# ZhenghaoFei/visual_odom

Hardware: NVIDIA H100
Metric: stereo frames/sec at 1241x376, 2000 feats; LK kernel HBM GB/s vs roofline (higher is better)
Workload: dtype u8/i32 fixed point + f32 (LK), f64 (pose)

## Files before the change

visual_odom_b200/csrc/ctx.cu:

```cuda
#include "ctx.h"
#include <string.h>
#include <stdlib.h>

void vo_set_error(vo_ctx* ctx, const char* fmt, ...)
{
    if (!ctx) return;
    va_list ap;
    va_start(ap, fmt);
    vsnprintf(ctx->err, sizeof(ctx->err), fmt, ap);
    va_end(ap);
}

extern "C" void vo_default_params(vo_params* p)
{
    p->fast_threshold = 20;
    p->fast_nonmax = 1;
    p->lk_win = 21;
    p->lk_max_level = 3;
    p->lk_max_iters = 30;
    p->lk_epsilon = 0.01;
    p->lk_min_eig = 0.001;
    p->circ_threshold = 0;
    p->pnp_iterations = 500;
    p->pnp_reproj_error = 0.5f;
// ... 260 lines not shown
    for (auto& p : ctx->pending)
        if (p.active) {
            VO_CUDA_CHECK(cudaEventSynchronize(p.done));
            p.active = false;
        }
    if (ctx->seq_inflight > 0 && ctx->side_stream[0]) VO_CUDA_CHECK(cudaStreamSynchronize(ctx->side_stream[0]));
    return VO_OK;
}

void vo_drop_graphs(vo_ctx* ctx)
{
    for (auto& g : ctx->graphs) cudaGraphExecDestroy(g.exec);
    ctx->graphs.clear();
}

void vo_set_calibration(vo_ctx* ctx, const float P_l[12], const float P_r[12])
{
    const bool same = ctx->have_P && memcmp(ctx->P_l, P_l, 12 * sizeof(float)) == 0 && memcmp(ctx->P_r, P_r, 12 * sizeof(float)) == 0;
    if (same) return;
    vo_drop_graphs(ctx);
    memcpy(ctx->P_l, P_l, 12 * sizeof(float));
    memcpy(ctx->P_r, P_r, 12 * sizeof(float));
    ctx->have_P = true;
}

void vo_free_state(vo_ctx* ctx)
{
    vo_drop_graphs(ctx);
    for (void* p : ctx->allocs) cudaFree(p);
    ctx->allocs.clear();
    if (ctx->d_seq_state) cudaFree(ctx->d_seq_state);
    ctx->d_seq_state = nullptr; ctx->seq_n_cap = 0;
    ctx->d_feat_pts = nullptr; ctx->d_feat_ages = nullptr; ctx->d_feat_cnt = ctx->d_bucket = ctx->d_seq_err = ctx->d_seq_live = nullptr;
    ctx->d_out = nullptr; ctx->out_stride = 0; ctx->out_per = 0;
    ctx->w = ctx->h = ctx->units = 0;
}

template <typename T>
static cudaError_t dalloc(vo_ctx* ctx, T** p, size_t count)
{
    void* q = nullptr;
    cudaError_t e = cudaMalloc(&q, count * sizeof(T) + 256);
    if (e == cudaSuccess) { ctx->allocs.push_back(q); *p = (T*)q; }
    return e;
}

typedef CUresult (*PFN_encodeTiled)(CUtensorMap*, CUtensorMapDataType, cuuint32_t, void*, const cuuint64_t*,
                                    const cuuint64_t*, const cuuint32_t*, const cuuint32_t*, CUtensorMapInterleave,
                                    CUtensorMapSwizzle, CUtensorMapL2promotion, CUtensorMapFloatOOBfill);

static int encode_maps(vo_ctx* ctx)
{
    void* fn = nullptr;
    cudaDriverEntryPointQueryResult qres;
    VO_CUDA_CHECK(cudaGetDriverEntryPoint("cuTensorMapEncodeTiled", &fn, cudaEnableDefault, &qres));
    if (!fn || qres != cudaDriverEntryPointSuccess) {
        vo_set_error(ctx, "cuTensorMapEncodeTiled not available from the driver");
        return VO_E_CUDA;
    }
    PFN_encodeTiled enc = (PFN_encodeTiled)fn;
    const int n_img = ctx->units * 4;
    for (int l = 0; l < ctx->pg.nlevels; l++) {
        const LevelGeom& g = ctx->pg.lv[l];
        {
            cuuint64_t dims[3] = {(cuuint64_t)g.pitch, (cuuint64_t)g.hp, (cuuint64_t)n_img};
            cuuint64_t strides[2] = {(cuuint64_t)g.pitch, (cuuint64_t)g.plane};
            cuuint32_t box_i[3] = {48, 22, 1}, box_j[3] = {48, 32, 1};
            cuuint32_t estr[3] = {1, 1, 1};
            CUresult r = enc(&ctx->maps.img_i[l], CU_TENSOR_MAP_DATA_TYPE_UINT8, 3, g.img, dims, strides, box_i, estr,
                             CU_TENSOR_MAP_INTERLEAVE_NONE, CU_TENSOR_MAP_SWIZZLE_NONE,
                             CU_TENSOR_MAP_L2_PROMOTION_NONE, CU_TENSOR_MAP_FLOAT_OOB_FILL_NONE);
            if (r == CUDA_SUCCESS)
                r = enc(&ctx->maps.img_j[l], CU_TENSOR_MAP_DATA_TYPE_UINT8, 3, g.img, dims, strides, box_j, estr,
                        CU_TENSOR_MAP_INTERLEAVE_NONE, CU_TENSOR_MAP_SWIZZLE_NONE,
                        CU_TENSOR_MAP_L2_PROMOTION_NONE, CU_TENSOR_MAP_FLOAT_OOB_FILL_NONE);
            if (r != CUDA_SUCCESS) { vo_set_error(ctx, "cuTensorMapEncodeTiled(u8 level %d) failed: %d", l, (int)r); return VO_E_CUDA; }
        }
        {
            cuuint64_t dims[3] = {(cuuint64_t)g.pitch, (cuuint64_t)g.hp, (cuuint64_t)n_img};
            cuuint64_t strides[2] = {(cuuint64_t)g.pitch * 4, (cuuint64_t)g.plane * 4};
            cuuint32_t box[3] = {28, 22, 1};
            cuuint32_t estr[3] = {1, 1, 1};
            CUresult r = enc(&ctx->maps.der[l], CU_TENSOR_MAP_DATA_TYPE_UINT32, 3, g.der, dims, strides, box, estr,
                             CU_TENSOR_MAP_INTERLEAVE_NONE, CU_TENSOR_MAP_SWIZZLE_NONE,
                             CU_TENSOR_MAP_L2_PROMOTION_NONE, CU_TENSOR_MAP_FLOAT_OOB_FILL_NONE);
            if (r != CUDA_SUCCESS) { vo_set_error(ctx, "cuTensorMapEncodeTiled(deriv level %d) failed: %d", l, (int)r); return VO_E_CUDA; }
        }
    }
    return VO_OK;
}

int vo_ensure_state(vo_ctx* ctx, int w, int h, int units, int )
{
    if (w <= 0 || h <= 0 || units <= 0) { vo_set_error(ctx, "bad geometry %dx%d units=%d", w, h, units); return VO_E_INVALID; }
    if (ctx->w == w && ctx->h == h && ctx->units >= units) return VO_OK;
    VO_CUDA_CHECK(cudaSetDevice(ctx->device));
    { int drc = vo_drain_pending(ctx); if (drc) return drc; }
    VO_CUDA_CHECK(cudaStreamSynchronize(ctx->stream));
    vo_free_state(ctx);
    const int n_img = units * 4;
    const int cap = ctx->cap;
    PyrGeom& pg = ctx->pg;
    memset(&pg, 0, sizeof(pg));
    int cw = w, ch = h;
    for (int l = 0; l <= ctx->p.lk_max_level; l++) {
        if (l > 0) {
            int nw = (cw + 1) / 2, nh = (ch + 1) / 2;
            if (nw <= VO_WIN || nh <= VO_WIN) break;
            cw = nw; ch = nh;
        }
        LevelGeom& g = pg.lv[l];
        g.w = cw; g.h = ch;
        g.pitch = ((cw + 2 * VO_PAD) + 63) / 64 * 64;
        g.hp = ch + 2 * VO_PAD;
        g.plane = (size_t)g.pitch * g.hp;
        VO_CUDA_CHECK(dalloc(ctx, &g.img, g.plane * n_img));
        VO_CUDA_CHECK(dalloc(ctx, &g.der, g.plane * n_img));
        VO_CUDA_CHECK(cudaMemsetAsync(g.img, 0, g.plane * n_img, ctx->stream));
        VO_CUDA_CHECK(cudaMemsetAsync(g.der, 0, g.plane * n_img * sizeof(uint32_t), ctx->stream));
        pg.nlevels = l + 1;
    }
    pg.n_img = n_img;
    VO_CUDA_CHECK(dalloc(ctx, &ctx->d_raw, (size_t)n_img * w * h));
    VO_CUDA_CHECK(dalloc(ctx, &ctx->d_raw_tab, (size_t)n_img));
    VO_CUDA_CHECK(dalloc(ctx, &ctx->d_ingest_tab, (size_t)n_img));
    {
        std::vector<const uint8_t*> tab(n_img);
        for (int i = 0; i < n_img; i++) tab[i] = ctx->d_raw + (size_t)i * w * h;
        VO_CUDA_CHECK(cudaMemcpyAsync(ctx->d_raw_tab, tab.data(), n_img * sizeof(uint8_t*), cudaMemcpyHostToDevice, ctx->stream));
        VO_CUDA_CHECK(cudaStreamSynchronize(ctx->stream));
    }
    const size_t uc = (size_t)units * cap;
    VO_CUDA_CHECK(dalloc(ctx, &ctx->d_pts_in, uc));
    VO_CUDA_CHECK(dalloc(ctx, &ctx->d_npts, (size_t)units));
    VO_CUDA_CHECK(dalloc(ctx, &ctx->d_pts_out, 4 * uc));
    VO_CUDA_CHECK(dalloc(ctx, &ctx->d_status, 4 * uc));
    VO_CUDA_CHECK(dalloc(ctx, &ctx->d_err, 4 * uc));
    VO_CUDA_CHECK(dalloc(ctx, &ctx->d_lk_progress, uc));
    VO_CUDA_CHECK(cudaMemsetAsync(ctx->d_lk_progress, 0, uc * sizeof(int), ctx->stream));
    VO_CUDA_CHECK(dalloc(ctx, &ctx->d_ages_in, uc));
    VO_CUDA_CHECK(dalloc(ctx, &ctx->d_ages_out, uc));
    VO_CUDA_CHECK(dalloc(ctx, &ctx->d_kept5, 5 * uc));
    VO_CUDA_CHECK(dalloc(ctx, &ctx->d_idx3, uc));
    VO_CUDA_CHECK(dalloc(ctx, &ctx->d_n3, (size_t)units));
    VO_CUDA_CHECK(dalloc(ctx, &ctx->d_valid4, 4 * uc));
    VO_CUDA_CHECK(dalloc(ctx, &ctx->d_idx5, uc));
    VO_CUDA_CHECK(dalloc(ctx, &ctx->d_n5, (size_t)units));
    {
        const long iw = w > 6 ? w - 6 : 0, ih = h > 6 ? h - 6 : 0;
        const long bound = ctx->p.fast_nonmax ? ((iw + 1) / 2) * ((ih + 1) / 2) : iw * ih;
        if (bound > (1L << 30)) { vo_set_error(ctx, "%dx%d: too many possible FAST corners", w, h); return VO_E_CAPACITY; }
        ctx->corner_cap = bound > 0 ? (int)bound : 1;
    }
    VO_CUDA_CHECK(dalloc(ctx, &ctx->d_score, (size_t)units * w * h));
    VO_CUDA_CHECK(dalloc(ctx, &ctx->d_rowbuf, (size_t)units * h * w));
    VO_CUDA_CHECK(dalloc(ctx, &ctx->d_rowcount, (size_t)units * h));
    VO_CUDA_CHECK(dalloc(ctx, &ctx->d_rowoff, (size_t)units * h));
    VO_CUDA_CHECK(dalloc(ctx, &ctx->d_ndet, (size_t)units));
    VO_CUDA_CHECK(dalloc(ctx, &ctx->d_corners, (size_t)units * ctx->corner_cap));
    VO_CUDA_CHECK(dalloc(ctx, &ctx->d_resp, (size_t)units * ctx->corner_cap));
    VO_CUDA_CHECK(dalloc(ctx, &ctx->d_want, (size_t)units));
    const size_t its = (size_t)ctx->p.pnp_iterations;
    VO_CUDA_CHECK(dalloc(ctx, &ctx->d_X, uc));
    VO_CUDA_CHECK(dalloc(ctx, &ctx->d_tprev, (size_t)units * 3));
    VO_CUDA_CHECK(dalloc(ctx, &ctx->d_pnp_state, (size_t)units));
    VO_CUDA_CHECK(dalloc(ctx, &ctx->d_subsets, (size_t)units * its * 5));
    VO_CUDA_CHECK(dalloc(ctx, &ctx->d_models, (size_t)units * its * 12));
    VO_CUDA_CHECK(dalloc(ctx, &ctx->d_counts, (size_t)units * its));
    VO_CUDA_CHECK(dalloc(ctx, &ctx->d_inliers, uc));
    VO_CUDA_CHECK(dalloc(ctx, &ctx->d_results, (size_t)units));
    ctx->feat_cap = ctx->corner_cap + cap;
    ctx->seq_active = false;
    VO_CUDA_CHECK(cudaMemsetAsync(ctx->d_results, 0, (size_t)units * sizeof(vo_unit_result_dev), ctx->stream));
    VO_CUDA_CHECK(cudaMemsetAsync(ctx->d_tprev, 0, (size_t)units * 3 * sizeof(double), ctx->stream));
    ctx->w = w; ctx->h = h; ctx->units = units;
    int rc = encode_maps(ctx);
    if (rc != VO_OK) { vo_free_state(ctx); return rc; }
    VO_CUDA_CHECK(cudaStreamSynchronize(ctx->stream));
    return VO_OK;
}

int vo_run_pyramid(vo_ctx* ctx, int plane0, int nplanes, cudaStream_t s)
{
    PyrGeom pg = ctx->pg;
    pg.n_img = nplanes;
    for (int l = 0; l < pg.nlevels; l++) {
        pg.lv[l].img += (size_t)plane0 * pg.lv[l].plane;
        pg.lv[l].der += (size_t)plane0 * pg.lv[l].plane;
    }
    ctx->launches += vo_launch_pyramid(pg, ctx->d_raw_tab + plane0, ctx->w, s);
    VO_CUDA_CHECK(cudaGetLastError());
    return VO_OK;
}

int vo_run_lk(vo_ctx* ctx, const View& v, int ncalls, const int* img_prev, const int* img_next, bool want_err)
{
    int rc = vo_run_pyramid(ctx, v.u0 * ctx->imgs_per_unit, v.n * ctx->imgs_per_unit, v.s);
    if (rc) return rc;
    return vo_run_lk_ring(ctx, v, ncalls, img_prev, img_next, want_err);
}

int vo_run_lk_ring(vo_ctx* ctx, const View& v, int ncalls, const int* img_prev, const int* img_next, bool want_err)
{
    const int ipu = ctx->imgs_per_unit;
    const size_t uo = (size_t)v.u0 * ctx->cap;
    const PyrGeom& pg = ctx->pg;

    LkArgs a;
    memset(&a, 0, sizeof(a));
    a.n_units = v.n;
    a.cap = ctx->cap;
    a.n_pts = ctx->d_npts + v.u0;
    a.imgs_per_unit = ipu;
    a.img_plane0 = v.plane0 >= 0 ? v.plane0 : v.u0 * ipu;
    a.ncalls = ncalls;
    for (int c = 0; c < ncalls; c++) { a.img_prev[c] = img_prev[c]; a.img_next[c] = img_next[c]; }
    a.nlevels = pg.nlevels;
    for (int l = 0; l < pg.nlevels; l++) { a.lw[l] = pg.lv[l].w; a.lh[l] = pg.lv[l].h; }
    a.max_iters = ctx->p.lk_max_iters;
    double eps = ctx->p.lk_epsilon;
    if (eps < 0.) eps = 0.; if (eps > 10.) eps = 10.;
    a.eps2 = eps * eps;
    a.min_eig = ctx->p.lk_min_eig;
    a.pts_in = ctx->d_pts_in + uo;
    a.pts_out = ctx->d_pts_out + uo;
    a.status_out = ctx->d_status + uo;
    a.err_out = want_err ? ctx->d_err + uo : nullptr;
    a.call_stride = (size_t)ctx->units * ctx->cap;
    a.use_tma = ctx->lk_use_tma ? 1 : 0;
    for (int l = 0; l < pg.nlevels; l++) {
        a.img_base[l] = ctx->pg.lv[l].img; a.der_base[l] = ctx->pg.lv[l].der;
        a.pitch[l] = pg.lv[l].pitch; a.plane[l] = pg.lv[l].plane;
    }

    cudaEvent_t e0 = nullptr, e1 = nullptr;
    if (ctx->lk_timing) {
        if (ctx->ev_used + 2 > ctx->ev_pool.size()) {
            cudaEvent_t a0, a1;
            VO_CUDA_CHECK(cudaEventCreate(&a0));
            VO_CUDA_CHECK(cudaEventCreate(&a1));
            ctx->ev_pool.push_back(a0); ctx->ev_pool.push_back(a1);
        }
        e0 = ctx->ev_pool[ctx->ev_used]; e1 = ctx->ev_pool[ctx->ev_used + 1];
        ctx->ev_used += 2;
        VO_CUDA_CHECK(cudaEventRecord(e0, v.s));
    }
    {
        size_t qi = 0;
        while (qi < ctx->lk_queue_streams.size() && ctx->lk_queue_streams[qi] != v.s) qi++;
        if (qi == ctx->lk_queue_streams.size()) {
            if (qi >= LK_QUEUES) { vo_set_error(ctx, "more than %d streams launch the LK kernel", LK_QUEUES); return VO_E_CAPACITY; }
            ctx->lk_queue_streams.push_back(v.s);
        }
        a.queue = ctx->d_lk_queue + 2 * qi;
        a.per_unit = ctx->lk_per_unit > 0 && ctx->lk_per_unit < ctx->cap ? ctx->lk_per_unit : ctx->cap;
        a.progress = ctx->d_lk_progress + uo;
        {
            int lk_sms = ctx->sm_count;
            for (int c = 0; c < VO_LANES; c++) if (ctx->part_on && v.s == ctx->part_lk_stream[c]) lk_sms = ctx->part_lk_sms;
            const long resident_warps = (long)lk_sms * vo_lk_ctas_per_sm(ctx->lk_ctas_per_sm) * LK_WARPS_PER_CTA;
            const bool big = (long)a.n_units * a.per_unit > resident_warps;
            a.span = ctx->lk_span > 0 ? ctx->lk_span : (big ? 2 : 0);
            a.quota = big ? ctx->lk_quota : 0;
        }
        int lk_sms = ctx->sm_count;
        for (int c = 0; c < VO_LANES; c++) if (ctx->part_on && v.s == ctx->part_lk_stream[c]) lk_sms = ctx->part_lk_sms;
        VO_CUDA_CHECK(vo_launch_lk_ring(ctx->maps, a, lk_sms, ctx->lk_ctas_per_sm, v.s));
    }
    ctx->launches += 1;
    if (e1) VO_CUDA_CHECK(cudaEventRecord(e1, v.s));
    return VO_OK;
}

int vo_run_filter(vo_ctx* ctx, const View& v, bool with_ages)
{
    const size_t uo = (size_t)v.u0 * ctx->cap;
    FilterArgs f;
    memset(&f, 0, sizeof(f));
    f.cap = ctx->cap;
    f.call_stride = (size_t)ctx->units * ctx->cap;
    f.circ_threshold = ctx->p.circ_threshold;
    f.n_pts = ctx->d_npts + v.u0;
    f.pts_in = ctx->d_pts_in + uo;
    f.pts_out = ctx->d_pts_out + uo;
    f.status = ctx->d_status + uo;
    f.ages_in = with_ages ? ctx->d_ages_in + uo : nullptr;
    f.ages_out = ctx->d_ages_out + uo;
    f.kept5 = ctx->d_kept5 + uo;
    f.idx3 = ctx->d_idx3 + uo;
    f.n3 = ctx->d_n3 + v.u0;
    f.valid4 = ctx->d_valid4 + uo;
    f.idx5 = ctx->d_idx5 + uo;
    f.n5 = ctx->d_n5 + v.u0;
    VO_CUDA_CHECK(vo_launch_ring_filter(f, v.n, v.s));
    ctx->launches += 1;
    return VO_OK;
}

int vo_run_fast(vo_ctx* ctx, const View& v, int plane_in_unit, bool want_resp)
{
    FastArgs a;
    memset(&a, 0, sizeof(a));
    const size_t plane = (size_t)ctx->w * ctx->h;
    a.n_units = v.n;
    a.img_tab = ctx->d_raw_tab + (size_t)(v.plane0 >= 0 ? v.plane0 : v.u0 * ctx->imgs_per_unit) + plane_in_unit;
    a.img_stride_idx = ctx->imgs_per_unit;
    a.w = ctx->w; a.h = ctx->h; a.pitch = ctx->w;
    a.threshold = ctx->p.fast_threshold; a.nonmax = ctx->p.fast_nonmax;
    a.score = ctx->d_score + v.u0 * plane; a.score_plane = plane;
    a.rowbuf = ctx->d_rowbuf + v.u0 * plane; a.rowcap = ctx->w;
    a.rowcount = ctx->d_rowcount + (size_t)v.u0 * ctx->h; a.rowoff = ctx->d_rowoff + (size_t)v.u0 * ctx->h;
    a.n_det = ctx->d_ndet + v.u0;
    a.corners = ctx->d_corners + (size_t)v.u0 * ctx->corner_cap;
    a.resp = want_resp ? ctx->d_resp + (size_t)v.u0 * ctx->corner_cap : nullptr;
    a.corner_cap = ctx->corner_cap;
    ctx->launches += vo_launch_fast(a, v.s);
    VO_CUDA_CHECK(cudaGetLastError());
    return VO_OK;
}

int vo_run_select(vo_ctx* ctx, const View& v)
{
    ctx->launches += vo_launch_select(ctx->d_corners + (size_t)v.u0 * ctx->corner_cap, ctx->corner_cap, ctx->d_ndet + v.u0,
                                      ctx->d_want + v.u0, ctx->d_pts_in + (size_t)v.u0 * ctx->cap, ctx->cap, ctx->d_npts + v.u0,
                                      v.n, v.s);
    VO_CUDA_CHECK(cudaGetLastError());
    return VO_OK;
}

int vo_run_triangulate(vo_ctx* ctx, const View& v, const float2* pts_l, const float2* pts_r, const int* n, float4* X4)
{
    const size_t uo = (size_t)v.u0 * ctx->cap;
    TriArgs t;
    memset(&t, 0, sizeof(t));
    t.cap = ctx->cap; t.n_pts = n + v.u0; t.pts_l = pts_l + uo; t.pts_r = pts_r + uo; t.X = ctx->d_X + uo; t.X4 = X4;
    for (int k = 0; k < 12; k++) { t.Pl[k] = (double)ctx->P_l[k]; t.Pr[k] = (double)ctx->P_r[k]; }
    ctx->launches += vo_launch_triangulate(t, v.n, v.s);
    VO_CUDA_CHECK(cudaGetLastError());
    return VO_OK;
}

int vo_run_pnp(vo_ctx* ctx, const View& v, const float2* pts2d, const int* n, const float* K9)
{
    const size_t uo = (size_t)v.u0 * ctx->cap, its = (size_t)ctx->p.pnp_iterations;
    PnpArgs a;
    memset(&a, 0, sizeof(a));
    a.n_units = v.n; a.cap = ctx->cap; a.iterations = ctx->p.pnp_iterations;
    a.n_pts = n + v.u0; a.X = ctx->d_X + uo; a.x = pts2d + uo;
    a.fu = (double)K9[0]; a.fv = (double)K9[4]; a.uc = (double)K9[2]; a.vc = (double)K9[5];
    const double thr = (double)ctx->p.pnp_reproj_error;
    a.thr2 = (float)(thr * thr);
    a.confidence = ctx->p.pnp_confidence;
    a.t_prev = ctx->d_tprev + (size_t)v.u0 * 3;
    a.state = ctx->d_pnp_state + v.u0; a.subsets = ctx->d_subsets + v.u0 * its * 5; a.models = ctx->d_models + v.u0 * its * 12;
    a.counts = ctx->d_counts + v.u0 * its;
    a.inliers = ctx->d_inliers + uo; a.results = ctx->d_results + v.u0;
    ctx->launches += vo_launch_pnp(a, v.s);
    VO_CUDA_CHECK(cudaGetLastError());
    return VO_OK;
}
```

visual_odom_b200/csrc/ctx.h:

```cpp
#pragma once
#include "common.cuh"
#include "lk_ring.h"
#include "filter.h"
#include "fast.h"
#include "pnp.h"
#include "seq.h"
#include "ess.h"
#include "../../include/vo_b200.h"
#include <vector>
#include <stdarg.h>
#define LK_QUEUES 32
#define VO_DIST_BUCKET 4
#define VO_DIST_NB 4
#define VO_LANES 3

struct vo_ctx {
    int device = 0;
    cudaStream_t own_stream = nullptr, stream = nullptr;
    vo_params p;
    char err[1024] = {0};
    long long launches = 0;
    int sm_count = 0;

    int w = 0, h = 0;
    int units = 0;
    int imgs_per_unit = 4;
    int cap = 0;
    PyrGeom pg;
    LkMaps maps;
    bool have_P = false;
    float P_l[12], P_r[12];

    uint8_t* d_raw = nullptr;
    const uint8_t** d_raw_tab = nullptr;
    vo_dimage* d_ingest_tab = nullptr;
    float2* d_pts_in = nullptr;
    int* d_npts = nullptr;
    float2* d_pts_out = nullptr;
    uint8_t* d_status = nullptr;
    float* d_err = nullptr;
    int* d_ages_in = nullptr;
    int* d_ages_out = nullptr;
    float2* d_kept5 = nullptr;
    int* d_idx3 = nullptr;
    int* d_n3 = nullptr;
    float2* d_valid4 = nullptr;
    int* d_idx5 = nullptr;
    int* d_n5 = nullptr;
    uint8_t* d_score = nullptr;
    uint16_t* d_rowbuf = nullptr;
    int* d_rowcount = nullptr;
    int* d_rowoff = nullptr;
    int* d_ndet = nullptr;
    float2* d_corners = nullptr;
    float* d_resp = nullptr;
    int* d_want = nullptr;
    int corner_cap = 0;
    float3* d_X = nullptr;
    double* d_tprev = nullptr;
    PnpState* d_pnp_state = nullptr;
    int* d_subsets = nullptr;
    double* d_models = nullptr;
    int* d_counts = nullptr;
    int* d_inliers = nullptr;
    vo_unit_result_dev* d_results = nullptr;
    float2* d_feat_pts = nullptr;
    int* d_feat_ages = nullptr;
    int* d_feat_cnt = nullptr;
    int* d_bucket = nullptr;
    int* d_seq_err = nullptr;
    int* d_seq_live = nullptr;
    void* d_seq_state = nullptr;
    int seq_n_cap = 0;
    int feat_cap = 0, bucket_cap = 4096;
    bool seq_active = false;
    bool seq_multi = false;
    int seq_n = 1;
    int seq_slot = 0;
    int seq_inflight = 0;
    long long seq_submitted = 0;
    int seq_channels[2] = {1, 1};
    cudaEvent_t seq_front_ev[2] = {nullptr, nullptr}, seq_back_ev[2] = {nullptr, nullptr};
    long long seq_frames = 0;
    std::vector<double> seq_pose;
    std::vector<char> seq_retired;
    std::vector<char> seq_live;
    uint8_t* d_bgr = nullptr;
    size_t bgr_bytes = 0;
    bool part_on = false;
    bool part_auto = true;
    bool part_pre_with_lk = false;
    int part_helper_sms = 0, part_lk_sms = 0;
    void* part_gctx[2] = {nullptr, nullptr};
    cudaStream_t part_lk_stream[VO_LANES] = {};
    cudaStream_t part_hp_stream[VO_LANES] = {};
    cudaEvent_t part_ev[VO_LANES][4] = {};
    void* dist_comm = nullptr;
    int dist_rank = 0, dist_world = 1;
    cudaStream_t dist_stream = nullptr, dist_snap_stream = nullptr;
    struct DistBucket { void* d = nullptr; void* h = nullptr; cudaEvent_t done = nullptr; int fill = 0, unwaited = 0, n_units = 0; bool flushed = false; };
    struct DistStep { int bucket = 0, index = 0; };
    DistBucket dist_bk[VO_DIST_NB];
    DistStep dist_steps[2 * VO_DIST_DEPTH];
    int dist_cur = 0;
    cudaEvent_t dist_ev_read = nullptr, dist_ev_fork = nullptr;
    size_t dist_bytes = 0;
    long long dist_head = 0, dist_tail = 0;
    void* d_ess = nullptr;
    int ess_cap = 0;
    bool mono_opt = false;
    bool seq_mono = false;
    void* d_seq_ess = nullptr;
    size_t seq_ess_bytes = 0;
    int seq_ess_cap = 0;
    cudaStream_t seq_mono_stream = nullptr;
    cudaEvent_t seq_mono_ev[2] = {nullptr, nullptr};
    std::vector<void*> allocs;

    void* h_pinned = nullptr;
    size_t h_pinned_bytes = 0;

    std::vector<cudaEvent_t> ev_pool;
    size_t ev_used = 0;
    double lk_ms = 0.0;
    long long lk_n = 0;
    bool lk_timing = true;
    bool lk_use_tma = true;
    int lk_ctas_per_sm = 0;
    int lk_quota = 0;
    int lk_span = 0;
    int* d_lk_progress = nullptr;
    int lk_per_unit = 0;
    int* d_lk_queue = nullptr;
    std::vector<cudaStream_t> lk_queue_streams;

    int batch_units = 0;
    int batch_uploaded = 0;
    bool batch_detect = false;
    int batch_streams = 2;
    bool use_graphs = true;
    struct RangeGraph { int u0, n; bool detect, tma; cudaStream_t s; int max_pts; cudaGraphExec_t exec; long long launches; };
    std::vector<RangeGraph> graphs;
    std::vector<int> slot_pts;
    cudaStream_t hi_stream[VO_LANES] = {};
    cudaEvent_t hi_ev[VO_LANES][4] = {};
    bool use_priorities = true;
    bool batch_graphs = false;
    cudaStream_t side_stream[VO_LANES] = {};
    cudaEvent_t fork_ev = nullptr, join_ev[VO_LANES] = {};
    struct Pending { int u0 = 0, n = 0; bool active = false; cudaEvent_t done = nullptr; };
    std::vector<Pending> pending;
    bool batch_outputs = false;
    uint8_t* d_out = nullptr;
    uint8_t* h_out = nullptr;
    size_t out_stride = 0;
    int out_per = 0, out_units = 0;
    unsigned submit_count = 0;
};

void vo_set_error(vo_ctx* ctx, const char* fmt, ...);
int vo_ensure_state(vo_ctx* ctx, int w, int h, int units, int imgs_per_unit);
void vo_free_state(vo_ctx* ctx);
void vo_drop_graphs(vo_ctx* ctx);
void vo_set_calibration(vo_ctx* ctx, const float P_l[12], const float P_r[12]);
int vo_drain_pending(vo_ctx* ctx);
int vo_partition_enable(vo_ctx* ctx, int helper_sms);
void vo_partition_destroy(vo_ctx* ctx);
int vo_dist_order_after_gathers(vo_ctx* ctx, cudaStream_t st);
void vo_dist_shutdown(vo_ctx* ctx);
int vo_claim_buffers(vo_ctx* ctx, const char* who, bool allow_pending_batches = false);
int vo_ensure_pinned(vo_ctx* ctx, size_t bytes);
int vo_ensure_bgr(vo_ctx* ctx, size_t bytes);
int vo_launch_bgr_to_gray(const vo_dimage* d_tab, const vo_dimage& packed, size_t packed_stride, uint8_t* d_gray, size_t img_stride_out,
                          int w, int h, int n_img, cudaStream_t s);
vo_dimage vo_packed_bgr(const uint8_t* d_bgr, int w);
int vo_check_dimage(vo_ctx* ctx, const char* who, const char* name, const vo_dimage* im, int w);
int vo_ingest_device(vo_ctx* ctx, const vo_dimage* h_tab, int n, int plane0, cudaStream_t st);
struct View { int u0, n; cudaStream_t s; int plane0 = -1; };
int vo_run_lk(vo_ctx* ctx, const View& v, int ncalls, const int* img_prev, const int* img_next, bool want_err);
int vo_run_pyramid(vo_ctx* ctx, int plane0, int nplanes, cudaStream_t s);
int vo_run_lk_ring(vo_ctx* ctx, const View& v, int ncalls, const int* img_prev, const int* img_next, bool want_err);
int vo_run_filter(vo_ctx* ctx, const View& v, bool with_ages);
int vo_run_fast(vo_ctx* ctx, const View& v, int plane_in_unit, bool want_resp);
int vo_run_select(vo_ctx* ctx, const View& v);
int vo_run_triangulate(vo_ctx* ctx, const View& v, const float2* pts_l, const float2* pts_r, const int* n, float4* X4 = nullptr);
int vo_run_pnp(vo_ctx* ctx, const View& v, const float2* pts2d, const int* n, const float* K9);
```

visual_odom_b200/csrc/fast.cu:

```cuda
#include "common.cuh"
#include "fast.h"

__global__ void __launch_bounds__(256) k_fast_score(const uint8_t* const* __restrict__ img_tab, int img_stride_idx,
                                                    int w, int h, int pitch, int threshold, int nonmax,
                                                    uint8_t* __restrict__ score, size_t score_plane)
{
    constexpr int ring_dx[16] = {0, 1, 2, 3, 3, 3, 2, 1, 0, -1, -2, -3, -3, -3, -2, -1};
    constexpr int ring_dy[16] = {3, 3, 2, 1, 0, -1, -2, -3, -3, -3, -2, -1, 0, 1, 2, 3};
    const int unit = blockIdx.z;
    const uint8_t* __restrict__ img = img_tab[unit * img_stride_idx];
    uint8_t* __restrict__ sc = score + (size_t)unit * score_plane;
    const int x = blockIdx.x * 32 + (threadIdx.x & 31);
    const int y = blockIdx.y * 8 + (threadIdx.x >> 5);
    if (x >= w || y >= h) return;
    int result = 0;
    if (x >= 3 && x < w - 3 && y >= 3 && y < h - 3) {
        const uint8_t* p = img + (size_t)y * pitch + x;
        const int v = p[0];
        float d[16];
        unsigned hi = 0, lo = 0;
#pragma unroll
        for (int k = 0; k < 16; k++) {
            const int r = p[ring_dy[k] * pitch + ring_dx[k]];
            d[k] = (float)(v - r);
            hi |= (unsigned)(r > v + threshold) << k;
            lo |= (unsigned)(r < v - threshold) << k;
        }
        unsigned mh = hi | (hi << 16), ml = lo | (lo << 16);
        mh &= mh >> 1; mh &= mh >> 2; mh &= mh >> 4; mh &= mh >> 1;
        ml &= ml >> 1; ml &= ml >> 2; ml &= ml >> 4; ml &= ml >> 1;
        if (mh | ml) {
            float mn[16], mx[16];
#pragma unroll
            for (int k = 0; k < 16; k++) { mn[k] = fminf(d[k], d[(k + 1) & 15]); mx[k] = fmaxf(d[k], d[(k + 1) & 15]); }
            float mn4[16], mx4[16];
#pragma unroll
            for (int k = 0; k < 16; k++) { mn4[k] = fminf(mn[k], mn[(k + 2) & 15]); mx4[k] = fmaxf(mx[k], mx[(k + 2) & 15]); }
            float A = -1000.f, B = 1000.f;
#pragma unroll
            for (int k = 0; k < 16; k++) {
                const float a8 = fminf(mn4[k], mn4[(k + 4) & 15]);
                const float b8 = fmaxf(mx4[k], mx4[(k + 4) & 15]);
                A = fmaxf(A, fminf(a8, d[(k + 8) & 15]));
                B = fminf(B, fmaxf(b8, d[(k + 8) & 15]));
            }
            result = max(threshold, (int)fmaxf(A, -B)) - 1;
            if (!nonmax) result = 1;
        }
    }
    sc[(size_t)y * w + x] = (uint8_t)result;
}

#define NMS_T 256
#define NMS_NC 8
__global__ void __launch_bounds__(NMS_T) k_fast_nms_row(const uint8_t* __restrict__ score, size_t score_plane, int w, int h,
                                                        int nonmax, uint16_t* __restrict__ rowbuf, int rowcap,
                                                        int* __restrict__ rowcount)
{
    const int y = blockIdx.x, unit = blockIdx.y;
    const uint8_t* __restrict__ sc = score + (size_t)unit * score_plane;
    uint16_t* __restrict__ out = rowbuf + ((size_t)unit * h + y) * rowcap;
    __shared__ uint8_t rows[3][NMS_T * NMS_NC + 2];
    __shared__ int wcnt[NMS_NC * (NMS_T / 32)];
    __shared__ int base;
    if (y < 3 || y >= h - 3) {
        if (threadIdx.x == 0) rowcount[unit * h + y] = 0;
        return;
    }
    if (threadIdx.x == 0) base = 0;
    const int lane = threadIdx.x & 31, warp = threadIdx.x >> 5;
    constexpr int NW = NMS_T / 32, SPAN = NMS_T * NMS_NC;
    for (int x0 = 0; x0 < w; x0 += SPAN) {
        for (int i = threadIdx.x; i < SPAN + 2; i += NMS_T) {
            const int x = x0 - 1 + i;
            const bool in = (x >= 0 && x < w);
            rows[0][i] = in ? sc[(size_t)(y - 1) * w + x] : 0;
            rows[1][i] = in ? sc[(size_t)y * w + x] : 0;
            rows[2][i] = in ? sc[(size_t)(y + 1) * w + x] : 0;
        }
        __syncthreads();
        unsigned bal[NMS_NC];
#pragma unroll
        for (int c = 0; c < NMS_NC; c++) {
            const int x = x0 + c * NMS_T + threadIdx.x, i = c * NMS_T + threadIdx.x + 1;
            bool keep = false;
            if (x < w) {
                const int s = rows[1][i];
                if (s > 0) {
                    keep = !nonmax ||
                           (s > rows[1][i - 1] && s > rows[1][i + 1] && s > rows[0][i - 1] && s > rows[0][i] &&
                            s > rows[0][i + 1] && s > rows[2][i - 1] && s > rows[2][i] && s > rows[2][i + 1]);
                }
            }
            bal[c] = __ballot_sync(0xffffffffu, keep);
            if (lane == 0) wcnt[c * NW + warp] = __popc(bal[c]);
        }
        __syncthreads();
        int carry_total = 0;
        if (threadIdx.x < NMS_NC * NW) {
            const int v = wcnt[threadIdx.x];
            int incl = v;
#pragma unroll
            for (int d = 1; d < 32; d <<= 1) {
                const int o = __shfl_up_sync(0xffffffffu, incl, d);
                if (lane >= d) incl += o;
            }
            carry_total = incl;
            wcnt[threadIdx.x] = incl - v;
        }
        __shared__ int w0_total, pass_total;
        if (threadIdx.x == 31) w0_total = carry_total;
        __syncthreads();
        if (threadIdx.x >= 32 && threadIdx.x < NMS_NC * NW) wcnt[threadIdx.x] += w0_total;
        if (threadIdx.x == NMS_NC * NW - 1) pass_total = carry_total + w0_total;
        __syncthreads();
        const int b0 = base;
#pragma unroll
        for (int c = 0; c < NMS_NC; c++) {
            if ((bal[c] >> lane) & 1u) {
                const int o = b0 + wcnt[c * NW + warp] + __popc(bal[c] & ((1u << lane) - 1u));
                if (o < rowcap) out[o] = (uint16_t)(x0 + c * NMS_T + threadIdx.x);
            }
        }
        __syncthreads();
        if (threadIdx.x == 0) base = b0 + pass_total;
        __syncthreads();
    }
    if (threadIdx.x == 0) rowcount[unit * h + y] = base < rowcap ? base : rowcap;
}

__global__ void __launch_bounds__(1024) k_fast_scan(const int* __restrict__ rowcount, int h, int* __restrict__ rowoff,
                                                    int* __restrict__ n_det)
{
    const int unit = blockIdx.x;
    const int* rc = rowcount + unit * h;
    int* ro = rowoff + unit * h;
    __shared__ int wsum[32];
    __shared__ int carry;
    if (threadIdx.x == 0) carry = 0;
    __syncthreads();
    const int lane = threadIdx.x & 31, warp = threadIdx.x >> 5;
    for (int y0 = 0; y0 < h; y0 += 1024) {
        const int y = y0 + threadIdx.x;
        int v = (y < h) ? rc[y] : 0;
        int incl = v;
#pragma unroll
        for (int d = 1; d < 32; d <<= 1) {
            int o = __shfl_up_sync(0xffffffffu, incl, d);
            if (lane >= d) incl += o;
        }
        if (lane == 31) wsum[warp] = incl;
        __syncthreads();
        int woff = carry;
        for (int k = 0; k < warp; k++) woff += wsum[k];
        if (y < h) ro[y] = woff + incl - v;
        __syncthreads();
        if (threadIdx.x == 0) {
            int t = 0;
            for (int k = 0; k < 32; k++) t += wsum[k];
            carry += t;
        }
        __syncthreads();
    }
    if (threadIdx.x == 0) n_det[unit] = carry;
}

__global__ void __launch_bounds__(128) k_fast_gather(const uint16_t* __restrict__ rowbuf, int rowcap,
                                                     const int* __restrict__ rowcount, const int* __restrict__ rowoff,
                                                     int h, const uint8_t* __restrict__ score, size_t score_plane, int w,
                                                     int nonmax, float2* __restrict__ out, float* __restrict__ resp, int cap)
{
    const int y = blockIdx.x, unit = blockIdx.y;
    const int n = rowcount[unit * h + y], off = rowoff[unit * h + y];
    const uint16_t* src = rowbuf + ((size_t)unit * h + y) * rowcap;
    for (int i = threadIdx.x; i < n; i += blockDim.x) {
        const int o = off + i;
        if (o < cap) {
            const int x = src[i];
            out[(size_t)unit * cap + o] = make_float2((float)x, (float)y);
            if (resp)
                resp[(size_t)unit * cap + o] = nonmax ? (float)score[(size_t)unit * score_plane + (size_t)y * w + x] : 0.f;
        }
    }
}

__global__ void k_select_stride(const float2* __restrict__ corners, int corner_cap, const int* __restrict__ n_det,
                                const int* __restrict__ want, float2* __restrict__ pts, int cap, int* __restrict__ n_pts)
{
    const int unit = blockIdx.y;
    int m = n_det[unit];
    if (m > corner_cap) m = corner_cap;
    int n = want[unit];
    if (n > cap) n = cap;
    if (n > m) n = m;
    const int i = blockIdx.x * blockDim.x + threadIdx.x;
    if (i == 0) n_pts[unit] = n;
    if (i >= n) return;
    const long idx = (n > 1) ? ((long)i * (m - 1)) / (n - 1) : 0;
    pts[(size_t)unit * cap + i] = corners[(size_t)unit * corner_cap + idx];
}

int vo_launch_fast(const FastArgs& a, cudaStream_t stream)
{
    dim3 g1((a.w + 31) / 32, (a.h + 7) / 8, a.n_units);
    k_fast_score<<<g1, 256, 0, stream>>>(a.img_tab, a.img_stride_idx, a.w, a.h, a.pitch, a.threshold, a.nonmax, a.score,
                                          a.score_plane);
    dim3 g2(a.h, a.n_units);
    k_fast_nms_row<<<g2, NMS_T, 0, stream>>>(a.score, a.score_plane, a.w, a.h, a.nonmax, a.rowbuf, a.rowcap, a.rowcount);
    k_fast_scan<<<a.n_units, 1024, 0, stream>>>(a.rowcount, a.h, a.rowoff, a.n_det);
    k_fast_gather<<<g2, 128, 0, stream>>>(a.rowbuf, a.rowcap, a.rowcount, a.rowoff, a.h, a.score, a.score_plane, a.w,
                                           a.nonmax, a.corners, a.resp, a.corner_cap);
    return 4;
}

int vo_launch_select(const float2* corners, int corner_cap, const int* n_det, const int* want, float2* pts, int cap,
                     int* n_pts, int n_units, cudaStream_t stream)
{
    dim3 g((cap + 255) / 256, n_units);
    k_select_stride<<<g, 256, 0, stream>>>(corners, corner_cap, n_det, want, pts, cap, n_pts);
    return 1;
}
```

visual_odom_b200/csrc/fast.h:

```cpp
#pragma once
#include "common.cuh"

struct FastArgs {
    int n_units;
    const uint8_t* const* img_tab;
    int img_stride_idx;
    int w, h, pitch;
    int threshold, nonmax;
    uint8_t* score;
    size_t score_plane;
    uint16_t* rowbuf;
    int rowcap;
    int* rowcount;
    int* rowoff;
    int* n_det;
    float2* corners;
    float* resp;
    int corner_cap;
};

int vo_launch_fast(const FastArgs& a, cudaStream_t stream);
int vo_launch_select(const float2* corners, int corner_cap, const int* n_det, const int* want, float2* pts, int cap,
                     int* n_pts, int n_units, cudaStream_t stream);
```

Before: 3847.

## Fuse FAST scoring and NMS into one banded shared-memory kernel

```diff
diff --git a/visual_odom_b200/csrc/ctx.cu b/visual_odom_b200/csrc/ctx.cu
--- a/visual_odom_b200/csrc/ctx.cu
+++ b/visual_odom_b200/csrc/ctx.cu
@@ -436,10 +436,10 @@
         if (bound > (1L << 30)) { vo_set_error(ctx, "%dx%d: too many possible FAST corners", w, h); return VO_E_CAPACITY; }
         ctx->corner_cap = bound > 0 ? (int)bound : 1;
     }
-    VO_CUDA_CHECK(dalloc(ctx, &ctx->d_score, (size_t)units * w * h));
-    VO_CUDA_CHECK(dalloc(ctx, &ctx->d_rowbuf, (size_t)units * h * w));
-    VO_CUDA_CHECK(dalloc(ctx, &ctx->d_rowcount, (size_t)units * h));
-    VO_CUDA_CHECK(dalloc(ctx, &ctx->d_rowoff, (size_t)units * h));
+    const size_t row_segs = (size_t)units * h * vo_fast_segments(w);
+    VO_CUDA_CHECK(dalloc(ctx, &ctx->d_rowbuf, row_segs * VO_FAST_SEG));
+    VO_CUDA_CHECK(dalloc(ctx, &ctx->d_rowcount, row_segs));
+    VO_CUDA_CHECK(dalloc(ctx, &ctx->d_rowoff, row_segs));
     VO_CUDA_CHECK(dalloc(ctx, &ctx->d_ndet, (size_t)units));
     VO_CUDA_CHECK(dalloc(ctx, &ctx->d_corners, (size_t)units * ctx->corner_cap));
     VO_CUDA_CHECK(dalloc(ctx, &ctx->d_resp, (size_t)units * ctx->corner_cap));
@@ -585,15 +585,14 @@
 {
     FastArgs a;
     memset(&a, 0, sizeof(a));
-    const size_t plane = (size_t)ctx->w * ctx->h;
+    const size_t row_segs = (size_t)ctx->h * vo_fast_segments(ctx->w);
     a.n_units = v.n;
     a.img_tab = ctx->d_raw_tab + (size_t)(v.plane0 >= 0 ? v.plane0 : v.u0 * ctx->imgs_per_unit) + plane_in_unit;
     a.img_stride_idx = ctx->imgs_per_unit;
     a.w = ctx->w; a.h = ctx->h; a.pitch = ctx->w;
     a.threshold = ctx->p.fast_threshold; a.nonmax = ctx->p.fast_nonmax;
-    a.score = ctx->d_score + v.u0 * plane; a.score_plane = plane;
-    a.rowbuf = ctx->d_rowbuf + v.u0 * plane; a.rowcap = ctx->w;
-    a.rowcount = ctx->d_rowcount + (size_t)v.u0 * ctx->h; a.rowoff = ctx->d_rowoff + (size_t)v.u0 * ctx->h;
+    a.rowbuf = ctx->d_rowbuf + v.u0 * row_segs * VO_FAST_SEG;
+    a.rowcount = ctx->d_rowcount + v.u0 * row_segs; a.rowoff = ctx->d_rowoff + v.u0 * row_segs;
     a.n_det = ctx->d_ndet + v.u0;
     a.corners = ctx->d_corners + (size_t)v.u0 * ctx->corner_cap;
     a.resp = want_resp ? ctx->d_resp + (size_t)v.u0 * ctx->corner_cap : nullptr;
diff --git a/visual_odom_b200/csrc/ctx.h b/visual_odom_b200/csrc/ctx.h
--- a/visual_odom_b200/csrc/ctx.h
+++ b/visual_odom_b200/csrc/ctx.h
@@ -47,8 +47,7 @@
     float2* d_valid4 = nullptr;
     int* d_idx5 = nullptr;
     int* d_n5 = nullptr;
-    uint8_t* d_score = nullptr;
-    uint16_t* d_rowbuf = nullptr;
+    uint32_t* d_rowbuf = nullptr;
     int* d_rowcount = nullptr;
     int* d_rowoff = nullptr;
     int* d_ndet = nullptr;
diff --git a/visual_odom_b200/csrc/fast.cu b/visual_odom_b200/csrc/fast.cu
--- a/visual_odom_b200/csrc/fast.cu
+++ b/visual_odom_b200/csrc/fast.cu
@@ -1,132 +1,172 @@
 #include "common.cuh"
 #include "fast.h"
-
-__global__ void __launch_bounds__(256) k_fast_score(const uint8_t* const* __restrict__ img_tab, int img_stride_idx,
-                                                    int w, int h, int pitch, int threshold, int nonmax,
-                                                    uint8_t* __restrict__ score, size_t score_plane)
+#include <cuda_fp16.h>
+
+#define FB_ROWS 8
+#define FB_T (32 * FB_ROWS)
+#define FB_CW VO_FAST_SEG
+#define FB_PR (FB_ROWS + 8)
+#define FB_PW (FB_CW + 16)
+#define FB_SR (FB_ROWS + 2)
+#define FB_SW (FB_CW + 8)
+#define FB_G (FB_SW / 4)
+
+static __device__ __forceinline__ uint32_t fb_shift(uint32_t w0, uint32_t w1, uint32_t w2, int dx)
+{
+    return dx < 0 ? __funnelshift_r(w0, w1, 8 * (4 + dx)) : (dx > 0 ? __funnelshift_r(w1, w2, 8 * dx) : w1);
+}
+
+__global__ void __launch_bounds__(FB_T, 5) k_fast_band(const uint8_t* const* __restrict__ img_tab, int img_stride_idx, int w,
+                                                    int h, int pitch, int threshold, int nonmax,
+                                                    uint32_t* __restrict__ rowbuf, int* __restrict__ rowcount)
 {
     constexpr int ring_dx[16] = {0, 1, 2, 3, 3, 3, 2, 1, 0, -1, -2, -3, -3, -3, -2, -1};
     constexpr int ring_dy[16] = {3, 3, 2, 1, 0, -1, -2, -3, -3, -3, -2, -1, 0, 1, 2, 3};
-    const int unit = blockIdx.z;
+    __shared__ __align__(16) uint32_t pix[FB_PR][FB_PW / 4];
+    __shared__ __align__(16) uint32_t scw[FB_SR][FB_G];
+    __shared__ uint16_t queue[FB_SR * FB_SW];
+    __shared__ int qn;
+    const int seg = blockIdx.x, nseg = gridDim.x, x0 = seg * FB_CW, y0 = blockIdx.y * FB_ROWS, unit = blockIdx.z;
     const uint8_t* __restrict__ img = img_tab[unit * img_stride_idx];
-    uint8_t* __restrict__ sc = score + (size_t)unit * score_plane;
-    const int x = blockIdx.x * 32 + (threadIdx.x & 31);
-    const int y = blockIdx.y * 8 + (threadIdx.x >> 5);
-    if (x >= w || y >= h) return;
-    int result = 0;
-    if (x >= 3 && x < w - 3 && y >= 3 && y < h - 3) {
-        const uint8_t* p = img + (size_t)y * pitch + x;
-        const int v = p[0];
-        float d[16];
-        unsigned hi = 0, lo = 0;
-#pragma unroll
-        for (int k = 0; k < 16; k++) {
-            const int r = p[ring_dy[k] * pitch + ring_dx[k]];
-            d[k] = (float)(v - r);
-            hi |= (unsigned)(r > v + threshold) << k;
-            lo |= (unsigned)(r < v - threshold) << k;
-        }
-        unsigned mh = hi | (hi << 16), ml = lo | (lo << 16);
-        mh &= mh >> 1; mh &= mh >> 2; mh &= mh >> 4; mh &= mh >> 1;
-        ml &= ml >> 1; ml &= ml >> 2; ml &= ml >> 4; ml &= ml >> 1;
-        if (mh | ml) {
-            float mn[16], mx[16];
-#pragma unroll
-            for (int k = 0; k < 16; k++) { mn[k] = fminf(d[k], d[(k + 1) & 15]); mx[k] = fmaxf(d[k], d[(k + 1) & 15]); }
-            float mn4[16], mx4[16];
-#pragma unroll
-            for (int k = 0; k < 16; k++) { mn4[k] = fminf(mn[k], mn[(k + 2) & 15]); mx4[k] = fmaxf(mx[k], mx[(k + 2) & 15]); }
-            float A = -1000.f, B = 1000.f;
+    const int lane = threadIdx.x & 31, warp = threadIdx.x >> 5;
+    const int Y = y0 + warp;
+    const uint32_t tt = (uint32_t)threshold * 0x01010101u;
+    const uint8_t* pb = reinterpret_cast<const uint8_t*>(&pix[0][0]);
+    uint8_t* sb = reinterpret_cast<uint8_t*>(&scw[0][0]);
+    if (threadIdx.x == 0) qn = 0;
+    constexpr int NWORD = FB_PR * (FB_PW / 4), NIT = (NWORD + FB_T - 1) / FB_T;
+    uint32_t lo[NIT], hi[NIT];
+    int sh[NIT];
+#pragma unroll
+    for (int it = 0; it < NIT; it++) {
+        const int i = threadIdx.x + it * FB_T;
+        const int pr = i / (FB_PW / 4), j = i % (FB_PW / 4);
+        const int yr = y0 - 4 + pr, X = x0 - 8 + 4 * j;
+        lo[it] = 0; hi[it] = 0; sh[it] = 0;
+        if (i < NWORD && yr >= 0 && yr < h) {
+            const uint8_t* row = img + (size_t)yr * pitch;
+            const uintptr_t a = reinterpret_cast<uintptr_t>(row + X);
+            const uintptr_t a0 = a & ~(uintptr_t)3;
+            const int s = (int)(a & 3);
+            if (X >= 0 && a0 >= reinterpret_cast<uintptr_t>(row) && a0 + (s ? 8 : 4) <= reinterpret_cast<uintptr_t>(row + w)) {
+                lo[it] = __ldg(reinterpret_cast<const uint32_t*>(a0));
+                if (s) hi[it] = __ldg(reinterpret_cast<const uint32_t*>(a0 + 4));
+                sh[it] = s;
+            } else {
+#pragma unroll
+                for (int b = 0; b < 4; b++)
+                    if (X + b >= 0 && X + b < w) lo[it] |= (uint32_t)__ldg(row + X + b) << (8 * b);
+            }
+        }
+    }
+#pragma unroll
+    for (int it = 0; it < NIT; it++) {
+        const int i = threadIdx.x + it * FB_T;
+        if (i < NWORD) pix[i / (FB_PW / 4)][i % (FB_PW / 4)] = __funnelshift_r(lo[it], hi[it], 8 * sh[it]);
+    }
+    __syncthreads();
+    for (int g0 = 0; g0 < FB_SR * FB_G; g0 += FB_T) {
+        const int gi = g0 + threadIdx.x;
+        const int sr = gi / FB_G, g = gi % FB_G;
+        const int yc = y0 - 1 + sr, xc = x0 - 4 + 4 * g;
+        unsigned cand = 0;
+        if (gi < FB_SR * FB_G && yc >= 3 && yc < h - 3 && xc + 3 >= 3 && xc < w - 3) {
+            uint32_t rw[7][3];
+#pragma unroll
+            for (int r = 0; r < 7; r++) {
+                rw[r][0] = pix[sr + r][g]; rw[r][1] = pix[sr + r][g + 1]; rw[r][2] = pix[sr + r][g + 2];
+            }
+            const uint32_t v = rw[3][1], vp = __vaddus4(v, tt), vm = __vsubus4(v, tt);
+            uint32_t hl = 0, hh = 0, ll = 0, lh = 0;
 #pragma unroll
             for (int k = 0; k < 16; k++) {
-                const float a8 = fminf(mn4[k], mn4[(k + 4) & 15]);
-                const float b8 = fmaxf(mx4[k], mx4[(k + 4) & 15]);
-                A = fmaxf(A, fminf(a8, d[(k + 8) & 15]));
-                B = fminf(B, fmaxf(b8, d[(k + 8) & 15]));
-            }
-            result = max(threshold, (int)fmaxf(A, -B)) - 1;
-            if (!nonmax) result = 1;
-        }
-    }
-    sc[(size_t)y * w + x] = (uint8_t)result;
-}
-
-#define NMS_T 256
-#define NMS_NC 8
-__global__ void __launch_bounds__(NMS_T) k_fast_nms_row(const uint8_t* __restrict__ score, size_t score_plane, int w, int h,
-                                                        int nonmax, uint16_t* __restrict__ rowbuf, int rowcap,
-                                                        int* __restrict__ rowcount)
-{
-    const int y = blockIdx.x, unit = blockIdx.y;
-    const uint8_t* __restrict__ sc = score + (size_t)unit * score_plane;
-    uint16_t* __restrict__ out = rowbuf + ((size_t)unit * h + y) * rowcap;
-    __shared__ uint8_t rows[3][NMS_T * NMS_NC + 2];
-    __shared__ int wcnt[NMS_NC * (NMS_T / 32)];
-    __shared__ int base;
-    if (y < 3 || y >= h - 3) {
-        if (threadIdx.x == 0) rowcount[unit * h + y] = 0;
-        return;
-    }
-    if (threadIdx.x == 0) base = 0;
-    const int lane = threadIdx.x & 31, warp = threadIdx.x >> 5;
-    constexpr int NW = NMS_T / 32, SPAN = NMS_T * NMS_NC;
-    for (int x0 = 0; x0 < w; x0 += SPAN) {
-        for (int i = threadIdx.x; i < SPAN + 2; i += NMS_T) {
-            const int x = x0 - 1 + i;
-            const bool in = (x >= 0 && x < w);
-            rows[0][i] = in ? sc[(size_t)(y - 1) * w + x] : 0;
-            rows[1][i] = in ? sc[(size_t)y * w + x] : 0;
-            rows[2][i] = in ? sc[(size_t)(y + 1) * w + x] : 0;
-        }
-        __syncthreads();
-        unsigned bal[NMS_NC];
-#pragma unroll
-        for (int c = 0; c < NMS_NC; c++) {
-            const int x = x0 + c * NMS_T + threadIdx.x, i = c * NMS_T + threadIdx.x + 1;
-            bool keep = false;
-            if (x < w) {
-                const int s = rows[1][i];
-                if (s > 0) {
-                    keep = !nonmax ||
-                           (s > rows[1][i - 1] && s > rows[1][i + 1] && s > rows[0][i - 1] && s > rows[0][i] &&
-                            s > rows[0][i + 1] && s > rows[2][i - 1] && s > rows[2][i] && s > rows[2][i + 1]);
-                }
-            }
-            bal[c] = __ballot_sync(0xffffffffu, keep);
-            if (lane == 0) wcnt[c * NW + warp] = __popc(bal[c]);
-        }
-        __syncthreads();
-        int carry_total = 0;
-        if (threadIdx.x < NMS_NC * NW) {
-            const int v = wcnt[threadIdx.x];
-            int incl = v;
-#pragma unroll
-            for (int d = 1; d < 32; d <<= 1) {
-                const int o = __shfl_up_sync(0xffffffffu, incl, d);
-                if (lane >= d) incl += o;
-            }
-            carry_total = incl;
-            wcnt[threadIdx.x] = incl - v;
-        }
-        __shared__ int w0_total, pass_total;
-        if (threadIdx.x == 31) w0_total = carry_total;
-        __syncthreads();
-        if (threadIdx.x >= 32 && threadIdx.x < NMS_NC * NW) wcnt[threadIdx.x] += w0_total;
-        if (threadIdx.x == NMS_NC * NW - 1) pass_total = carry_total + w0_total;
-        __syncthreads();
-        const int b0 = base;
-#pragma unroll
-        for (int c = 0; c < NMS_NC; c++) {
-            if ((bal[c] >> lane) & 1u) {
-                const int o = b0 + wcnt[c * NW + warp] + __popc(bal[c] & ((1u << lane) - 1u));
-                if (o < rowcap) out[o] = (uint16_t)(x0 + c * NMS_T + threadIdx.x);
-            }
-        }
-        __syncthreads();
-        if (threadIdx.x == 0) base = b0 + pass_total;
-        __syncthreads();
-    }
-    if (threadIdx.x == 0) rowcount[unit * h + y] = base < rowcap ? base : rowcap;
+                const int r = 3 + ring_dy[k];
+                const uint32_t rk = fb_shift(rw[r][0], rw[r][1], rw[r][2], ring_dx[k]);
+                const uint32_t mh = __vcmpgtu4(rk, vp) & 0x01010101u, ml = __vcmpltu4(rk, vm) & 0x01010101u;
+                if (k < 8) { hl |= mh << k; ll |= ml << k; }
+                else       { hh |= mh << (k - 8); lh |= ml << (k - 8); }
+            }
+#pragma unroll
+            for (int b = 0; b < 4; b++) {
+                const unsigned hi = ((hl >> (8 * b)) & 255u) | (((hh >> (8 * b)) & 255u) << 8);
+                const unsigned lo = ((ll >> (8 * b)) & 255u) | (((lh >> (8 * b)) & 255u) << 8);
+                unsigned mh = hi | (hi << 16), ml = lo | (lo << 16);
+                mh &= mh >> 1; mh &= mh >> 2; mh &= mh >> 4; mh &= mh >> 1;
+                ml &= ml >> 1; ml &= ml >> 2; ml &= ml >> 4; ml &= ml >> 1;
+                const int x = xc + b;
+                if ((mh | ml) && x >= 3 && x < w - 3) cand |= 1u << b;
+            }
+        }
+        if (gi < FB_SR * FB_G) scw[sr][g] = nonmax ? 0u : (((cand & 1u) ? 1u : 0u) | ((cand & 2u) ? 1u << 8 : 0u) |
+                                                            ((cand & 4u) ? 1u << 16 : 0u) | ((cand & 8u) ? 1u << 24 : 0u));
+        if (nonmax) {
+            unsigned bal[4];
+            int tot = 0;
+#pragma unroll
+            for (int b = 0; b < 4; b++) { bal[b] = __ballot_sync(0xffffffffu, (cand >> b) & 1u); tot += __popc(bal[b]); }
+            int qb = 0;
+            if (lane == 0 && tot) qb = atomicAdd(&qn, tot);
+            qb = __shfl_sync(0xffffffffu, qb, 0);
+            const unsigned lt = (1u << lane) - 1u;
+#pragma unroll
+            for (int b = 0; b < 4; b++) {
+                if ((cand >> b) & 1u) queue[qb + __popc(bal[b] & lt)] = (uint16_t)(sr * FB_SW + 4 * g + b);
+                qb += __popc(bal[b]);
+            }
+        }
+    }
+    __syncthreads();
+    if (nonmax) {
+        const int n = qn;
+        for (int q = 2 * threadIdx.x; q < n; q += 2 * FB_T) {
+            const int ia = queue[q], ib = queue[q + 1 < n ? q + 1 : q];
+            const uint8_t* pa = pb + (ia / FB_SW + 3) * FB_PW + ia % FB_SW + 4;
+            const uint8_t* pq = pb + (ib / FB_SW + 3) * FB_PW + ib % FB_SW + 4;
+            const int va = pa[0], vb = pq[0];
+            __half2 d[16];
+#pragma unroll
+            for (int k = 0; k < 16; k++) {
+                const int o = ring_dy[k] * FB_PW + ring_dx[k];
+                d[k] = __halves2half2(__int2half_rn(va - (int)pa[o]), __int2half_rn(vb - (int)pq[o]));
+            }
+            __half2 mn[16], mx[16];
+#pragma unroll
+            for (int k = 0; k < 16; k++) { mn[k] = __hmin2(d[k], d[(k + 1) & 15]); mx[k] = __hmax2(d[k], d[(k + 1) & 15]); }
+            __half2 mn4[16], mx4[16];
+#pragma unroll
+            for (int k = 0; k < 16; k++) { mn4[k] = __hmin2(mn[k], mn[(k + 2) & 15]); mx4[k] = __hmax2(mx[k], mx[(k + 2) & 15]); }
+            __half2 A = __float2half2_rn(-1000.f), B = __float2half2_rn(1000.f);
+#pragma unroll
+            for (int k = 0; k < 16; k++) {
+                const __half2 a8 = __hmin2(mn4[k], mn4[(k + 4) & 15]);
+                const __half2 b8 = __hmax2(mx4[k], mx4[(k + 4) & 15]);
+                A = __hmax2(A, __hmin2(a8, d[(k + 8) & 15]));
+                B = __hmin2(B, __hmax2(b8, d[(k + 8) & 15]));
+            }
+            const float2 Af = __half22float2(A), Bf = __half22float2(B);
+            sb[ia] = (uint8_t)(max(threshold, (int)fmaxf(Af.x, -Bf.x)) - 1);
+            if (q + 1 < n) sb[ib] = (uint8_t)(max(threshold, (int)fmaxf(Af.y, -Bf.y)) - 1);
+        }
+        __syncthreads();
+    }
+    int base = 0;
+    if (Y < h) {
+        uint32_t* __restrict__ out = rowbuf + (((size_t)unit * h + Y) * nseg + seg) * FB_CW;
+        const uint8_t* s1 = sb + (warp + 1) * FB_SW + 4;
+#pragma unroll
+        for (int c = 0; c < FB_CW / 32; c++) {
+            const int xo = 32 * c + lane, X = x0 + xo;
+            const int s = s1[xo];
+            const bool keep = X < w && s > 0 &&
+                              (!nonmax || (s > s1[xo - 1] && s > s1[xo + 1] && s > s1[xo - FB_SW - 1] && s > s1[xo - FB_SW] &&
+                                           s > s1[xo - FB_SW + 1] && s > s1[xo + FB_SW - 1] && s > s1[xo + FB_SW] &&
+                                           s > s1[xo + FB_SW + 1]));
+            const unsigned b = __ballot_sync(0xffffffffu, keep);
+            if (keep) out[base + __popc(b & ((1u << lane) - 1u))] = (uint32_t)X | ((uint32_t)s << 16);
+            base += __popc(b);
+        }
+    }
+    if (lane == 0 && Y < h) rowcount[((size_t)unit * h + Y) * nseg + seg] = base;
 }
 
 __global__ void __launch_bounds__(1024) k_fast_scan(const int* __restrict__ rowcount, int h, int* __restrict__ rowoff,
@@ -165,21 +205,23 @@
     if (threadIdx.x == 0) n_det[unit] = carry;
 }
 
-__global__ void __launch_bounds__(128) k_fast_gather(const uint16_t* __restrict__ rowbuf, int rowcap,
-                                                     const int* __restrict__ rowcount, const int* __restrict__ rowoff,
-                                                     int h, const uint8_t* __restrict__ score, size_t score_plane, int w,
-                                                     int nonmax, float2* __restrict__ out, float* __restrict__ resp, int cap)
-{
-    const int y = blockIdx.x, unit = blockIdx.y;
-    const int n = rowcount[unit * h + y], off = rowoff[unit * h + y];
-    const uint16_t* src = rowbuf + ((size_t)unit * h + y) * rowcap;
-    for (int i = threadIdx.x; i < n; i += blockDim.x) {
-        const int o = off + i;
-        if (o < cap) {
-            const int x = src[i];
-            out[(size_t)unit * cap + o] = make_float2((float)x, (float)y);
-            if (resp)
-                resp[(size_t)unit * cap + o] = nonmax ? (float)score[(size_t)unit * score_plane + (size_t)y * w + x] : 0.f;
+__global__ void __launch_bounds__(128) k_fast_gather(const uint32_t* __restrict__ rowbuf, const int* __restrict__ rowcount,
+                                                     const int* __restrict__ rowoff, int nseg, int h, int nonmax,
+                                                     float2* __restrict__ out, float* __restrict__ resp, int cap)
+{
+    const int y = blockIdx.x, unit = blockIdx.y, lane = threadIdx.x & 31;
+    for (int sg = threadIdx.x >> 5; sg < nseg; sg += blockDim.x >> 5) {
+        const size_t i0 = ((size_t)unit * h + y) * nseg + sg;
+        const int n = rowcount[i0], off = rowoff[i0];
+        const uint32_t* src = rowbuf + i0 * VO_FAST_SEG;
+        for (int i = lane; i < n; i += 32) {
+            const int o = off + i;
+            if (o < cap) {
+                const uint32_t e = src[i];
+                out[(size_t)unit * cap + o] = make_float2((float)(e & 0xffffu), (float)y);
+                if (resp)
+                    resp[(size_t)unit * cap + o] = nonmax ? (float)(e >> 16) : 0.f;
+            }
         }
     }
 }
@@ -202,15 +244,15 @@
 
 int vo_launch_fast(const FastArgs& a, cudaStream_t stream)
 {
-    dim3 g1((a.w + 31) / 32, (a.h + 7) / 8, a.n_units);
-    k_fast_score<<<g1, 256, 0, stream>>>(a.img_tab, a.img_stride_idx, a.w, a.h, a.pitch, a.threshold, a.nonmax, a.score,
-                                          a.score_plane);
+    const int nseg = vo_fast_segments(a.w);
+    dim3 g1(nseg, (a.h + FB_ROWS - 1) / FB_ROWS, a.n_units);
+    k_fast_band<<<g1, FB_T, 0, stream>>>(a.img_tab, a.img_stride_idx, a.w, a.h, a.pitch, a.threshold, a.nonmax, a.rowbuf,
+                                          a.rowcount);
+    k_fast_scan<<<a.n_units, 1024, 0, stream>>>(a.rowcount, a.h * nseg, a.rowoff, a.n_det);
     dim3 g2(a.h, a.n_units);
-    k_fast_nms_row<<<g2, NMS_T, 0, stream>>>(a.score, a.score_plane, a.w, a.h, a.nonmax, a.rowbuf, a.rowcap, a.rowcount);
-    k_fast_scan<<<a.n_units, 1024, 0, stream>>>(a.rowcount, a.h, a.rowoff, a.n_det);
-    k_fast_gather<<<g2, 128, 0, stream>>>(a.rowbuf, a.rowcap, a.rowcount, a.rowoff, a.h, a.score, a.score_plane, a.w,
-                                           a.nonmax, a.corners, a.resp, a.corner_cap);
-    return 4;
+    k_fast_gather<<<g2, 128, 0, stream>>>(a.rowbuf, a.rowcount, a.rowoff, nseg, a.h, a.nonmax, a.corners, a.resp,
+                                           a.corner_cap);
+    return 3;
 }
 
 int vo_launch_select(const float2* corners, int corner_cap, const int* n_det, const int* want, float2* pts, int cap,
diff --git a/visual_odom_b200/csrc/fast.h b/visual_odom_b200/csrc/fast.h
--- a/visual_odom_b200/csrc/fast.h
+++ b/visual_odom_b200/csrc/fast.h
@@ -1,5 +1,8 @@
 #pragma once
 #include "common.cuh"
+
+#define VO_FAST_SEG 256
+static inline int vo_fast_segments(int w) { return (w + VO_FAST_SEG - 1) / VO_FAST_SEG; }
 
 struct FastArgs {
     int n_units;
@@ -7,10 +10,7 @@
     int img_stride_idx;
     int w, h, pitch;
     int threshold, nonmax;
-    uint8_t* score;
-    size_t score_plane;
-    uint16_t* rowbuf;
-    int rowcap;
+    uint32_t* rowbuf;
     int* rowcount;
     int* rowoff;
     int* n_det;
```

Result: no change. 3874, median of 6 (+0.7%).
